# optozorax/portal

Hardware: AMD Instinct MI355X
Metric: Mray/s (primary rays) + ms/frame at 3840x2160, portal_in_portal depth=40 (higher is better)
Workload: dtype f32; 1 GPU; scenes/portal_in_portal.ron 3840x2160 aa=1 depth=40; build=w4, affine_rays=True, candidate_frames_identical=True, frames_in_flight=2, parallelism=row-block interleave x1, jit_specialisation=all scene uniforms baked (camera dynamic)

## Files before the change

### include/portal_amd.h

```cpp
#ifndef PORTAL_AMD_H
#define PORTAL_AMD_H

#include <stddef.h>
#include <stdint.h>

#ifdef __cplusplus
extern "C" {
#endif

#define PTL_OK 0
#define PTL_UNKNOWN_UNIFORM 1
#define PTL_ERR_INVALID (-1)
#define PTL_ERR_COMPILE (-2)
#define PTL_ERR_HIP (-3)
#define PTL_ERR_TYPE (-4)
#define PTL_ERR_SCENE (-5)
#define PTL_ERR_NO_DEVICE (-6)

const char* ptl_last_error(void);

const char* ptl_version(void);

int ptl_device_count(void);

// ... 20 lines not shown

int ptl_kernel_set_uniform(ptl_kernel* k, const char* name, ptl_type type, const void* value);

int ptl_kernel_set_texture(ptl_kernel* k, const char* sampler, const uint8_t* rgba8, int width, int height);

typedef struct {
    int width, height;
    int rb_phase, rb_stride;
    int in_place;
} ptl_frame;

int ptl_frame_shard_rows(const ptl_frame* f);

int ptl_kernel_render(ptl_kernel* k, const ptl_frame* frame, void* out_rgba8, void* out_rgba32f, void* segments,
                      void* stream, float* elapsed_ms);

int ptl_kernel_render_to_host(ptl_kernel* k, const ptl_frame* frame, uint8_t* host_rgba8, float* host_rgba32f,
                              uint64_t* host_segments, float* elapsed_ms);
int ptl_kernel_max_slices(ptl_kernel* k);
int ptl_kernel_stage_slice(ptl_kernel* k, int index);
int ptl_kernel_stage_slice_from(ptl_kernel* k, int index, const void* block, size_t size);
int ptl_kernel_hold_textures(ptl_kernel* k, int hold);
size_t ptl_kernel_uniform_block_size(ptl_kernel* k);
int ptl_kernel_snapshot_uniforms(ptl_kernel* k, void* dst, size_t cap);
int ptl_kernel_render_slices(ptl_kernel* k, const ptl_frame* frame, int n, void* out_rgba8, void* out_rgba32f, unsigned long long slice_pixels,
                             void* stream, float* elapsed_ms);

int ptl_kernel_teleport_ray(ptl_kernel* k, const float a[3], const float b[3], float out_pos[3], int* hit_object,
                            int* changed_subspace, int* teleported);
int ptl_kernel_prebuild_teleport(ptl_kernel* k);
// ... 45 lines not shown
#define PTL_FLAG_NO_FIRST_TRIP (1u << 13)
#define PTL_FLAG_EXACT_CR (1u << 14)
#define PTL_FLAG_NO_UNROLL (1u << 15)
#define PTL_FLAG_NO_FIRST_TRIP_PLANES (1u << 16)
#define PTL_FLAG_ASYNC_REJIT (1u << 17)
#define PTL_FLAG_QUICK_JIT (1u << 18)
#define PTL_FLAG_NO_ZERO_MASKS (1u << 19)
#define PTL_FLAG_SPECIALIZE_PATTERNS (1u << 20)
#define PTL_FLAG_BOUNDED_SNIPPETS (1u << 21)
#define PTL_FLAG_SLICES (1u << 22)
#define PTL_FLAG_NO_AFFINE_RAYS (1u << 23)
#define PTL_FLAG_KEEP_TRANSFORM_DODGES (1u << 24)
#define PTL_FLAG_CHECK_AFFINE (1u << 25)
#define PTL_FLAG_MATERIAL_TABLE_LDS (1u << 26)
#define PTL_FLAG_MATERIAL_TABLE_SCALAR (1u << 27)

int ptl_scene_generate_source(ptl_scene* s, unsigned flags, char** source);
int ptl_scene_generated_defines(ptl_scene* s, char* out, size_t cap);
int ptl_scene_zero_mask_probes(ptl_scene* s, int* reused, int* probed);
int ptl_scene_uniform_layout(ptl_scene* s, const ptl_uniform_desc** descs, int* n, size_t* block_size);
int ptl_scene_set_uniforms(ptl_scene* s, ptl_kernel* k);
typedef void (*ptl_uniform_cb)(void* user, const char* name, ptl_type type, const void* value);
int ptl_scene_visit_uniforms(ptl_scene* s, ptl_uniform_cb cb, void* user);
int ptl_scene_source_line_owner(ptl_scene* s, int line, char* kind, size_t kind_cap, char* name, size_t name_cap,
                                int* local_line);
void ptl_free(void* p);

int ptl_renderer_create(ptl_scene* s, int device, const char* asset_root, unsigned flags, ptl_renderer** out, char* log,
                        size_t log_cap);
int ptl_renderer_create_with_options(ptl_scene* s, int device, const char* asset_root, unsigned flags, const char* const* option_names,
// ... 103 lines not shown
```

### portal_amd/__init__.py

```python
from __future__ import annotations

import ctypes as C
import os
from typing import Callable, Optional

import numpy as np

_HERE = os.path.dirname(os.path.abspath(__file__))
REPO_ROOT = os.path.dirname(_HERE)
LIB_PATH = os.path.join(_HERE, "libportal_amd.so")

os.environ.setdefault("PTL_CACHE_DIR", os.path.join(_HERE, "_cache"))



def _share_torch_hip_runtime() -> None:
    if "PTL_HIP_LIB" in os.environ:
        return
    import importlib.util

    try:
        spec = importlib.util.find_spec("torch")
    except (ImportError, ValueError):
        spec = None
# ... 10 lines not shown
FLAG_SPECIALIZE_INTS = 1
FLAG_COUNT_SEGMENTS = 2
FLAG_SPECIALIZE_ALL = 4
FLAG_SPECIALIZE_STATIC = 8
FLAG_ANAGLYPH = 16
FLAG_NO_DERIVED_UNIFORMS = 32
FLAG_NO_FIRST_TRIP = 8192
FLAG_NO_UNIFORM_HOIST = 4096
FLAG_NO_DEFERRED_UPDATES = 128
FLAG_QUICK_JIT = 262144
FLAG_SPECIALIZE_PATTERNS = 1048576
FLAG_BOUNDED_SNIPPETS = 2097152
FLAG_KEEP_TRANSFORM_DODGES = 16777216
FLAG_MATERIAL_TABLE_LDS = 1 << 26
FLAG_MATERIAL_TABLE_SCALAR = 1 << 27
FLAG_CHECK_AFFINE = 1 << 25
FLAG_NO_AFFINE_RAYS = 8388608
FLAG_SLICES = 4194304
FLAG_NO_ZERO_MASKS = 524288
FLAG_ASYNC_REJIT = 131072
FLAG_NO_FIRST_TRIP_PLANES = 65536
FLAG_NO_UNROLL = 32768
FLAG_EXACT_CR = 16384
FLAG_FAST_MATH = 64


def flag_waves(n: int) -> int:
    return (int(n) & 0xF) << 8


class PortalError(RuntimeError):
    pass


class UniformDesc(C.Structure):
    _fields_ = [("name", C.c_char_p), ("type", C.c_int), ("offset", C.c_size_t)]


class CalculatedCam(C.Structure):
# ... 8 lines not shown


def _load() -> C.CDLL:
    if not os.path.exists(LIB_PATH):
        raise PortalError(f"{LIB_PATH} is missing: run `python -c 'import __graft_entry__ as g; g.build()'` or `make`")
    lib = C.CDLL(LIB_PATH)
    vp, cp, ci, cd, cs = C.c_void_p, C.c_char_p, C.c_int, C.c_double, C.c_size_t
    P = C.POINTER
    sig = {
        "ptl_last_error": (cp, []),
        "ptl_version": (cp, []),
        "ptl_device_count": (ci, []),
        "ptl_kernel_compile": (ci, [ci, cp, P(UniformDesc), ci, cs, P(cp), ci, P(vp), cp, cs]),
        "ptl_kernel_code_object": (ci, [vp, P(vp), P(cs)]),
        "ptl_kernel_resources": (ci, [vp, P(ci), P(ci), P(ci)]),
        "ptl_kernel_set_uniform": (ci, [vp, cp, ci, vp]),
        "ptl_kernel_set_texture": (ci, [vp, cp, vp, ci, ci]),
        "ptl_frame_shard_rows": (ci, [P(Frame)]),
        "ptl_kernel_render": (ci, [vp, P(Frame), vp, vp, vp, vp, P(C.c_float)]),
        "ptl_kernel_render_to_host": (ci, [vp, P(Frame), vp, vp, P(C.c_uint64), P(C.c_float)]),
        "ptl_kernel_teleport_ray": (ci, [vp, P(C.c_float), P(C.c_float), P(C.c_float), P(ci), P(ci), P(ci)]),
        "ptl_kernel_destroy": (None, [vp]),
        "ptl_scene_load_file": (ci, [cp, P(vp)]),
        "ptl_scene_load_text": (ci, [cp, P(vp)]),
        "ptl_scene_free": (None, [vp]),
        "ptl_scene_set_uniform": (ci, [vp, cp, cd]),
        "ptl_scene_set_time": (ci, [vp, cd, cd]),
        "ptl_scene_set_trefoil": (ci, [vp, cp, cp]),
        "ptl_scene_get_trefoil": (ci, [vp, cp, cp, cs]),
        "ptl_scene_init_stage": (ci, [vp, cp, cp, cs]),
# ... 378 lines not shown

    def teleport_external_ray(self, a, b):
        pa_, pb_, out = (C.c_double * 3)(*a), (C.c_double * 3)(*b), (C.c_double * 3)()
        hit, sub, tel = C.c_int(), C.c_int(), C.c_int()
        _check(lib().ptl_renderer_teleport_ray(self._h, pa_, pb_, out, C.byref(hit), C.byref(sub), C.byref(tel)), "teleport_external_ray")
        return (tuple(out) if tel.value else None), bool(hit.value), bool(sub.value)

    def prebuild_teleport(self) -> None:
        _check(lib().ptl_renderer_prebuild_teleport(self._h), "prebuild_teleport")

    def resources(self) -> dict:
        regs, scratch, lds = C.c_int(), C.c_int(), C.c_int()
        _check(lib().ptl_kernel_resources(lib().ptl_renderer_kernel(self._h), C.byref(regs), C.byref(scratch), C.byref(lds)), "kernel_resources")
        return {"registers": regs.value, "scratch_bytes": scratch.value, "lds_bytes": lds.value}

    def move_camera(self, look_at, alpha: float, beta: float, r: float):
        la, tel, blk = (C.c_double * 3)(*look_at), C.c_int(), C.c_int()
        _check(lib().ptl_renderer_move_camera(self._h, la, alpha, beta, r, C.byref(tel), C.byref(blk)), "move_camera")
        return bool(tel.value), bool(blk.value)

    def update(self, seconds: float):
        tel, blk = C.c_int(), C.c_int()
        _check(lib().ptl_renderer_update(self._h, float(seconds), C.byref(tel), C.byref(blk)), "update")
        return bool(tel.value), bool(blk.value)

    def rejit_count(self) -> int:
        return lib().ptl_renderer_rejit_count(self._h)

    def affine_rays(self) -> bool:
        lib().ptl_renderer_kernel(self._h)
# ... 315 lines not shown
```

### portal_amd/csrc/device/ptl_entry.h

```cpp

#if defined(PTL_NO_TELEPORT_ENTRY) && !defined(PTL_NO_DERIVE_ENTRY)
#define PTL_NO_DERIVE_ENTRY
#endif

#if PTL_DEVICE_BUILD

#ifdef PTL_WAVES_PER_EU
#define PTL_LAUNCH_BOUNDS __launch_bounds__(256, PTL_WAVES_PER_EU)
#else
#define PTL_LAUNCH_BOUNDS __launch_bounds__(256)
#endif

#if !defined(PTL_TELEPORT_MODULE)
extern "C" __global__ void PTL_LAUNCH_BOUNDS
ptl_render_kernel(unsigned int* __restrict__ out_rgba8,
                  float* __restrict__ out_rgba32f,
                  int width, int height,
                  int rb_phase, int rb_stride,
                  unsigned long long* __restrict__ segment_counter,
                  int in_place) {
#ifndef PTL_DIRECT_STORE
    __shared__ unsigned int tile[8][32 + 1];
#endif
    const int t = (int)threadIdx.x;
    const int wave = t >> 6, lane = t & 63;
    const int lx = wave * 8 + (lane & 7);
    const int ly = lane >> 3;
#ifdef PTL_XCD_SWIZZLE
// ... 167 lines not shown
```

### portal_amd/csrc/host/capi.cpp

```cpp
#include <chrono>
#include <cmath>
#include <cstdlib>
#include <cstring>
#include <map>
#include <memory>
#include <mutex>
#include <dirent.h>

#include <algorithm>
#include <atomic>
#include <set>
#include <thread>
#include <string>
#include <vector>

#include "../../../include/portal_amd.h"
#include "codegen.h"
#include "formula.h"
#include "glsl_hoist.h"
#include "glsl_translate.h"
#include "internal.h"
#include "scene.h"

using namespace ptl;
// ... 431 lines not shown
static KernelOptions options_from_flags(unsigned flags) {
    auto on = [flags](unsigned bit) { return (flags & bit) != 0; };
    KernelOptions o;
    o.specialize_ints = on(PTL_FLAG_SPECIALIZE_INTS);
    o.count_segments = on(PTL_FLAG_COUNT_SEGMENTS);
    o.specialize_all = on(PTL_FLAG_SPECIALIZE_ALL);
    o.anaglyph = on(PTL_FLAG_ANAGLYPH);
    o.specialize_static = on(PTL_FLAG_SPECIALIZE_STATIC);
    o.specialize_static_ints = on(PTL_FLAG_SPECIALIZE_PATTERNS);
    o.derived_uniforms = !on(PTL_FLAG_NO_DERIVED_UNIFORMS);
    o.fast_math = on(PTL_FLAG_FAST_MATH);
    o.exact_cr = on(PTL_FLAG_EXACT_CR);
    o.quick_jit = on(PTL_FLAG_QUICK_JIT) && !o.specialize_static;
    o.mask_zero_elements = specialised(flags) && !on(PTL_FLAG_NO_ZERO_MASKS);
    o.slices_entry = on(PTL_FLAG_SLICES);
    o.bound_snippets = on(PTL_FLAG_BOUNDED_SNIPPETS);
    const bool first_trip_forms = on(PTL_FLAG_KEEP_TRANSFORM_DODGES) || specialised(flags);
    o.first_trip_planes = first_trip_forms && !on(PTL_FLAG_NO_FIRST_TRIP_PLANES);
    if (const char* ab = std::getenv("PTL_AB_FIRST_TRIP_PLANES"); ab && (ab[0] == '0' || ab[0] == '1')) o.first_trip_planes = ab[0] == '1' && !on(PTL_FLAG_NO_FIRST_TRIP_PLANES);
    if (const char* skip = std::getenv("PTL_AFFINE_RAYS_SKIP_SCAN")) o.skip_affine_scan = skip[0] == '1';
    o.unroll_baked_loops = !on(PTL_FLAG_NO_UNROLL) && !o.quick_jit;
    o.keep_transform_dodges = on(PTL_FLAG_KEEP_TRANSFORM_DODGES);
    o.material_table = on(PTL_FLAG_MATERIAL_TABLE_SCALAR) ? 2 : (on(PTL_FLAG_MATERIAL_TABLE_LDS) ? 1 : 0);
    o.check_affine = on(PTL_FLAG_CHECK_AFFINE);
    o.affine_rays = !on(PTL_FLAG_NO_AFFINE_RAYS);
    o.first_trip = first_trip_forms && !on(PTL_FLAG_NO_FIRST_TRIP);
    o.hoist_uniform_work = !on(PTL_FLAG_NO_UNIFORM_HOIST);
    return o;
}

// ... 1394 lines not shown
```

### portal_amd/csrc/host/codegen.cpp

```cpp
#include "codegen.h"
#include "glsl_hoist.h"
#include "glsl_tokens.h"

#include <cstdlib>
#include <cstring>

#include <algorithm>
#include <charconv>
#include <cmath>
#include <cstdio>
#include <regex>
#include <set>
#include <sstream>
#include <tuple>

namespace ptl {

void LineNumbersByKey::offset(int lines) {
    for (auto& kv : ranges) {
        kv.second.start += lines;
        kv.second.end += lines;
    }
}
void LineNumbersByKey::add(const ElementKey& key, LineRange r) {
// ... 1463 lines not shown
    slots["uniforms"] = emit_uniforms(scene, plan, opts);
    std::tie(slots["material_processing"], slots["materials_defines"]) = emit_materials(scene, plan, opts);
    slots["intersection_functions"] = emit_intersection_functions(scene, plan, opts);
    slots["intersections"] = emit_intersections(scene, plan, opts, false);
    slots["intersections_first"] = plan.first_trip_plane_tests > 0 ? emit_intersections(scene, plan, opts, true) : StringStorage();
    slots["derive"] = emit_derive(scene, plan, opts);
    slots["intersection_material_functions"] = emit_intersection_material_functions(scene, plan, opts);
    slots["intersection_material_processing"] = emit_intersection_material_processing(scene, plan, opts, false);
    slots["intersection_material_processing_first"] = emit_intersection_material_processing(scene, plan, opts, true);
    slots["library"] = emit_library(scene, plan, opts);
    slots["predefined_library"] = emit_predefined_library(scene, plan, opts);
    slots["skybox_processing"] = emit_skybox_processing(scene, plan, opts);

    StringStorage body = apply_template(device_source_trace_template(), std::move(slots));
    body.add_string("\n");
    body.add_string(device_source_entry());
    GeneratedKernel gk = describe_kernel(plan, opts);
    gk.source = std::move(body.storage);
    gk.line_numbers = std::move(body.line_numbers);
    apply_zero_masks(gk.source, gk.masked);
    if (opts.slices_entry) apply_slices_entry(gk.source);
    return gk;
}

}
```

### portal_amd/csrc/host/codegen.h

```cpp
#pragma once
#include <map>
#include <set>
#include <string>
#include <vector>

#include "glsl_translate.h"
#include "scene.h"

namespace ptl {

struct ElementKey {
    std::string kind;
    std::string name;
    bool operator<(const ElementKey& o) const { return kind != o.kind ? kind < o.kind : name < o.name; }
    bool operator==(const ElementKey& o) const { return kind == o.kind && name == o.name; }
};
struct LineRange {
    int start = 0, end = 0;
};

class LineNumbersByKey {
public:
    std::map<ElementKey, LineRange> ranges;
    void offset(int lines);
// ... 54 lines not shown
    bool specialize_static = false;
    std::set<std::string> keep_dynamic;
    std::map<std::string, int> baked_options;
    bool mask_zero_elements = false;
    std::set<std::string> keep_unmasked;
    ZeroMaskCache* mask_cache = nullptr;
    bool full_chains = false;
    bool derived_uniforms = true;
    bool hoist_uniform_work = true;
    bool first_trip = true;
    bool unroll_baked_loops = true;
    bool exact_cr = false;
    bool first_trip_planes = true;
    bool bound_snippets = false;
    bool slices_entry = false;
    bool affine_rays = true;
    bool check_affine = false;
    bool skip_affine_scan = false;
    int material_table = 0;
    bool keep_transform_dodges = false;
    bool quick_jit = false;
    bool fast_math = false;
};

struct DerivedPlane {
    int object = 0, side = 0;
    std::string member;
    std::string normal_expr;
    std::string arg_expr;
};
// ... 42 lines not shown
```

### portal_amd/csrc/host/hip_api.cpp

```cpp
#ifndef _GNU_SOURCE
#define _GNU_SOURCE
#endif
#include "hip_api.h"

#include <stdlib.h>

#include <dlfcn.h>
#include <link.h>

#include <cstdlib>
#include <cstring>
#include <mutex>
#include <vector>

namespace ptl::hip {
namespace {

std::string loaded_library_path(const char* stem) {
    struct Ctx {
        const char* stem;
        std::string found;
    } ctx{stem, ""};
    dl_iterate_phdr(
        [](struct dl_phdr_info* info, size_t, void* data) -> int {
// ... 71 lines not shown
const Runtime* runtime(std::string* error) {
    static std::mutex mu;
    static Runtime rt;
    static bool tried = false, ok = false;
    static std::string err;
    std::lock_guard<std::mutex> lock(mu);
    if (!tried) {
        tried = true;
        const char* env = std::getenv("PTL_HIP_LIB");
        std::vector<std::string> candidates = {env ? env : "", loaded_library_path("libamdhip64.so"), "libamdhip64.so",
                                               "/opt/rocm/lib/libamdhip64.so"};
        void* h = open_first(candidates, &rt.path, &err);
        if (h) {
            ok = bind(h, "hipInit", rt.hipInit, &err) && bind(h, "hipGetDeviceCount", rt.hipGetDeviceCount, &err) &&
                 bind(h, "hipSetDevice", rt.hipSetDevice, &err) && bind(h, "hipGetDevice", rt.hipGetDevice, &err) &&
                 bind(h, "hipMalloc", rt.hipMalloc, &err) && bind(h, "hipFree", rt.hipFree, &err) &&
                 bind(h, "hipHostMalloc", rt.hipHostMalloc, &err) && bind(h, "hipHostFree", rt.hipHostFree, &err) &&
                 bind(h, "hipMemcpy", rt.hipMemcpy, &err) && bind(h, "hipMemcpyAsync", rt.hipMemcpyAsync, &err) &&
                 bind(h, "hipMemsetAsync", rt.hipMemsetAsync, &err) && bind(h, "hipStreamSynchronize", rt.hipStreamSynchronize, &err) &&
                 bind(h, "hipDeviceSynchronize", rt.hipDeviceSynchronize, &err) &&
                 bind(h, "hipStreamCreateWithFlags", rt.hipStreamCreateWithFlags, &err) && bind(h, "hipStreamDestroy", rt.hipStreamDestroy, &err) &&
                 bind(h, "hipStreamWaitEvent", rt.hipStreamWaitEvent, &err) && bind(h, "hipEventCreateWithFlags", rt.hipEventCreateWithFlags, &err) && bind(h, "hipEventCreate", rt.hipEventCreate, &err) &&
                 bind(h, "hipEventDestroy", rt.hipEventDestroy, &err) && bind(h, "hipEventRecord", rt.hipEventRecord, &err) &&
                 bind(h, "hipEventSynchronize", rt.hipEventSynchronize, &err) &&
                 bind(h, "hipEventElapsedTime", rt.hipEventElapsedTime, &err) && bind(h, "hipModuleLoadData", rt.hipModuleLoadData, &err) &&
                 bind(h, "hipModuleUnload", rt.hipModuleUnload, &err) && bind(h, "hipModuleGetFunction", rt.hipModuleGetFunction, &err) &&
                 bind(h, "hipModuleGetGlobal", rt.hipModuleGetGlobal, &err) && bind(h, "hipFuncGetAttribute", rt.hipFuncGetAttribute, &err) &&
                 bind(h, "hipModuleLaunchKernel", rt.hipModuleLaunchKernel, &err) && bind(h, "hipGetErrorString", rt.hipGetErrorString, &err) &&
                 bind(h, "hipIpcGetMemHandle", rt.hipIpcGetMemHandle, &err) && bind(h, "hipIpcOpenMemHandle", rt.hipIpcOpenMemHandle, &err) &&
                 bind(h, "hipIpcCloseMemHandle", rt.hipIpcCloseMemHandle, &err) && bind(h, "hipGetLastError", rt.hipGetLastError, &err) &&
// ... 63 lines not shown
```

### portal_amd/csrc/host/hip_api.h

```cpp
#pragma once
#include <cstddef>
#include <string>

namespace ptl::hip {

using hipError_t = int;
using hipStream_t = void*;
using hipEvent_t = void*;
using hipModule_t = void*;
using hipFunction_t = void*;
using hipDeviceptr_t = void*;
using hiprtcProgram = void*;
using hiprtcResult = int;

struct IpcMemHandle {
    char reserved[64];
};

struct Runtime {
    std::string path;
    hipError_t (*hipInit)(unsigned);
    hipError_t (*hipGetDeviceCount)(int*);
    hipError_t (*hipSetDevice)(int);
    hipError_t (*hipGetDevice)(int*);
    hipError_t (*hipMalloc)(void**, size_t);
    hipError_t (*hipFree)(void*);
    hipError_t (*hipHostMalloc)(void**, size_t, unsigned);
    hipError_t (*hipHostFree)(void*);
    hipError_t (*hipMemcpy)(void*, const void*, size_t, int);
    hipError_t (*hipMemcpyAsync)(void*, const void*, size_t, int, hipStream_t);
    hipError_t (*hipMemsetAsync)(void*, int, size_t, hipStream_t);
    hipError_t (*hipStreamSynchronize)(hipStream_t);
    hipError_t (*hipStreamCreateWithFlags)(hipStream_t*, unsigned);
    hipError_t (*hipStreamDestroy)(hipStream_t);
    hipError_t (*hipStreamWaitEvent)(hipStream_t, hipEvent_t, unsigned);
    hipError_t (*hipEventCreateWithFlags)(hipEvent_t*, unsigned);
    hipError_t (*hipDeviceSynchronize)();
    hipError_t (*hipEventCreate)(hipEvent_t*);
    hipError_t (*hipEventDestroy)(hipEvent_t);
// ... 5 lines not shown
    hipError_t (*hipModuleGetFunction)(hipFunction_t*, hipModule_t, const char*);
    hipError_t (*hipModuleGetGlobal)(hipDeviceptr_t*, size_t*, hipModule_t, const char*);
    hipError_t (*hipFuncGetAttribute)(int*, int, hipFunction_t);
    hipError_t (*hipModuleLaunchKernel)(hipFunction_t, unsigned, unsigned, unsigned, unsigned, unsigned, unsigned, unsigned,
                                        hipStream_t, void**, void**);
    const char* (*hipGetErrorString)(hipError_t);
    hipError_t (*hipIpcGetMemHandle)(IpcMemHandle*, void*);
    hipError_t (*hipIpcOpenMemHandle)(void**, IpcMemHandle, unsigned);
    hipError_t (*hipIpcCloseMemHandle)(void*);
    hipError_t (*hipGetLastError)();
    hipError_t (*hipDeviceCanAccessPeer)(int*, int, int);
    hipError_t (*hipDeviceEnablePeerAccess)(int, unsigned);
    hipError_t (*hipMemcpy2DAsync)(void*, size_t, const void*, size_t, size_t, size_t, int, hipStream_t);
};
constexpr int kFuncAttrSharedSizeBytes = 1, kFuncAttrLocalSizeBytes = 3, kFuncAttrNumRegs = 4;
constexpr unsigned kStreamNonBlocking = 1, kEventDisableTiming = 2, kIpcMemLazyEnablePeerAccess = 1;
constexpr int kMemcpyHostToDevice = 1;
constexpr int kMemcpyDeviceToHost = 2;
constexpr int kMemcpyDefault = 4;
constexpr int kErrorPeerAccessAlreadyEnabled = 704;

struct Rtc {
    std::string path;
    std::string real_path;
    hiprtcResult (*hiprtcCreateProgram)(hiprtcProgram*, const char*, const char*, int, const char**, const char**);
    hiprtcResult (*hiprtcCompileProgram)(hiprtcProgram, int, const char**);
    hiprtcResult (*hiprtcGetProgramLogSize)(hiprtcProgram, size_t*);
    hiprtcResult (*hiprtcGetProgramLog)(hiprtcProgram, char*);
    hiprtcResult (*hiprtcGetCodeSize)(hiprtcProgram, size_t*);
    hiprtcResult (*hiprtcGetCode)(hiprtcProgram, char*);
// ... 28 lines not shown
```

### portal_amd/csrc/host/kernel.cpp

```cpp
#include <sys/stat.h>
#include <unistd.h>

#include <cstdio>
#include <cstdlib>
#include <cstring>
#include <atomic>
#include <fstream>
#include <iterator>
#include <memory>
#include <map>
#include <string>
#include <vector>

#include "../../../include/portal_amd.h"
#include "hip_api.h"
#include "internal.h"

namespace ptl {

thread_local std::string g_last_error;
void set_last_error(const std::string& msg) { g_last_error = msg; }

namespace {

// ... 138 lines not shown
    std::vector<void*> retired_textures;
    bool staged_since_launch = false;
    int texture_holds = 0;
    hip::hipEvent_t ev0 = nullptr, ev1 = nullptr;
    hip::hipEvent_t ev_done = nullptr;
    bool sliced = false;
    bool affine_rays = false;
    hip::hipFunction_t derive_slices_fn = nullptr;
    void* dev_slices = nullptr;
    std::vector<unsigned char> staged;
    bool slice0_dirty = true;
    bool split = false;
    std::string source;
    std::vector<std::string> defines;
    ptl_kernel* companion = nullptr;
    unsigned block_waves = 4;
    void* last_stream = nullptr;
    bool launched = false;
};

extern "C" const char* ptl_last_error(void) { return g_last_error.c_str(); }

extern "C" const char* ptl_version(void) {
    static std::string v;
    std::string e1, e2;
    const hip::Runtime* rt = hip::runtime(&e1);
    const hip::Rtc* rc = hip::rtc(&e2);
    std::string toolchain = "?";
    if (rc) {
        size_t so = rc->real_path.rfind(".so.");
// ... 10 lines not shown
    if (rt->hipGetDeviceCount(&n) != 0) return 0;
    return n;
}

static constexpr int kMaxSlices = 16;

static size_t type_size(ptl_type t) {
    switch (t) {
        case PTL_MAT4: return 64;
        case PTL_F32: case PTL_I32: return 4;
        case PTL_VEC2: return 8;
        case PTL_VEC3: return 12;
        case PTL_SAMPLER: return 16;
    }
    return 0;
}

static thread_local bool tl_skip_cache_read = false;
static thread_local const std::vector<char>* tl_prebuilt_code = nullptr;

extern "C" int ptl_kernel_compile_prebuilt(int device, const char* hip_source, const ptl_uniform_desc* uniforms, int n_uniforms, size_t uniform_block_size,
                                           const char* const* defines, int n_defines, const void* code, size_t code_size, ptl_kernel** out, char* log,
                                           size_t log_cap) {
    if (!code || code_size < 64) return PTL_ERR_INVALID;
    const std::vector<char> copy(static_cast<const char*>(code), static_cast<const char*>(code) + code_size);
    tl_prebuilt_code = &copy;
    const int rc = ptl_kernel_compile(device, hip_source, uniforms, n_uniforms, uniform_block_size, defines, n_defines, out, log, log_cap);
    tl_prebuilt_code = nullptr;
    return rc;
}
// ... 11 lines not shown
    k->device = device;
    for (int i = 0; i < n_uniforms; ++i) {
        k->slots[uniforms[i].name] = {uniforms[i].type, uniforms[i].offset};
        if (uniforms[i].offset + type_size(uniforms[i].type) > uniform_block_size) {
            set_last_error(std::string("uniform `") + uniforms[i].name + "` lies outside the block");
            return PTL_ERR_INVALID;
        }
    }
    k->shadow.assign(uniform_block_size, 0);

    bool teleport_only = false;
    for (int i = 0; i < n_defines; ++i) {
        if (std::string(defines[i]) == "PTL_AFFINE_RAYS") k->affine_rays = true;
        if (std::string(defines[i]) == "PTL_RENDER_MODULE") k->split = true;
        if (std::string(defines[i]) == "PTL_TELEPORT_MODULE") teleport_only = true;
    }
    if (k->split) {
        k->source = hip_source;
        for (int i = 0; i < n_defines; ++i) k->defines.push_back(defines[i]);
    }
    std::vector<std::string> opts = compile_options(defines, n_defines);
    std::string cdir = cache_dir();
    std::string cache_path;
    if (!cdir.empty()) {
        unsigned long long h = fnv1a(hip_source);
        for (auto& o : opts) h = fnv1a(o, h);
        h = fnv1a("jit policy 6: occupancy retries end with an -O1 attempt", h);
        std::string err;
        if (const hip::Rtc* rc = hip::rtc(&err)) {
            h = fnv1a("hiprtc " + rc->real_path, h);
// ... 139 lines not shown
    }
    if (rt->hipModuleGetFunction(&k->derive_fn, k->module, "ptl_derive_kernel") != 0) {
        k->derive_fn = nullptr;
        rt->hipGetLastError();
    }
    if (!hip_ok(rt, rt->hipModuleGetGlobal(&k->dev_block, &k->dev_block_size, k->module, "_ZN4glsl5ptl_uE"), "hipModuleGetGlobal(ptl_u)"))
        return PTL_ERR_HIP;
    if (k->dev_block_size < uniform_block_size) {
        set_last_error("uniform block in the code object is smaller than the declared layout");
        return PTL_ERR_INVALID;
    }
    rt->hipEventCreate(&k->ev0);
    rt->hipEventCreate(&k->ev1);
    rt->hipEventCreateWithFlags(&k->ev_done, hip::kEventDisableTiming);
    if (const char* e = std::getenv("PTL_BLOCK_WAVES")) k->block_waves = (e[0] == '1' || e[0] == '2') ? (unsigned)(e[0] - '0') : 4u;
    *out = k.release();
    return PTL_OK;
}

extern "C" int ptl_kernel_clone(ptl_kernel* src, ptl_kernel** out) {
    if (!src || !out) return PTL_ERR_INVALID;
    if (src->device < 0 || !src->fn) return PTL_ERR_NO_DEVICE;
    const hip::Runtime* rt = hip::runtime(nullptr);
    if (!rt) return PTL_ERR_NO_DEVICE;
    auto k = std::make_unique<ptl_kernel>();
    k->device = src->device;
    k->code = src->code;
    k->slots = src->slots;
    k->shadow = src->shadow;
    k->block_waves = src->block_waves;
    k->split = src->split;
    k->source = src->source;
    k->defines = src->defines;
    if (!hip_ok(rt, rt->hipSetDevice(k->device), "hipSetDevice")) return PTL_ERR_HIP;
    if (!hip_ok(rt, rt->hipModuleLoadData(&k->module, k->code.data()), "hipModuleLoadData(clone)")) return PTL_ERR_HIP;
    auto fail = [&](int rc) {
        rt->hipModuleUnload(k->module);
        k->module = nullptr;
        return rc;
    };
    if (rt->hipModuleGetFunction(&k->fn, k->module, src->sliced ? "ptl_render_slices_kernel" : "ptl_render_kernel") != 0 ||
        (src->sliced && rt->hipModuleGetFunction(&k->derive_slices_fn, k->module, "ptl_derive_slices_kernel") != 0)) {
        hip_ok(rt, 1, "hipModuleGetFunction(clone)");
        return fail(PTL_ERR_HIP);
    }
    k->sliced = src->sliced;
    if (rt->hipModuleGetFunction(&k->teleport_fn, k->module, "ptl_teleport_kernel") != 0) {
        k->teleport_fn = nullptr;
        rt->hipGetLastError();
    }
    if (rt->hipModuleGetFunction(&k->derive_fn, k->module, "ptl_derive_kernel") != 0) {
        k->derive_fn = nullptr;
        rt->hipGetLastError();
    }
    if (!hip_ok(rt, rt->hipModuleGetGlobal(&k->dev_block, &k->dev_block_size, k->module, "_ZN4glsl5ptl_uE"), "hipModuleGetGlobal(ptl_u)")) return fail(PTL_ERR_HIP);
    rt->hipEventCreate(&k->ev0);
    rt->hipEventCreate(&k->ev1);
    rt->hipEventCreateWithFlags(&k->ev_done, hip::kEventDisableTiming);
    k->dirty = true;
    *out = k.release();
    return PTL_OK;
}

extern "C" int ptl_kernel_copy_uniforms(ptl_kernel* dst, const ptl_kernel* src) {
    if (!dst || !src || dst->shadow.size() != src->shadow.size()) return PTL_ERR_INVALID;
    if (std::memcmp(dst->shadow.data(), src->shadow.data(), src->shadow.size()) != 0) {
        dst->shadow = src->shadow;
        dst->dirty = true;
        dst->slice0_dirty = true;
    }
    return PTL_OK;
}

extern "C" int ptl_kernel_code_object(ptl_kernel* k, const void** data, size_t* size) {
    if (!k) return PTL_ERR_INVALID;
    if (data) *data = k->code.data();
    if (size) *size = k->code.size();
// ... 232 lines not shown
    if (k->device < 0 || !k->fn) return PTL_ERR_NO_DEVICE;
    const hip::Runtime* rt = hip::runtime(nullptr);
    if (!hip_ok(rt, rt->hipSetDevice(k->device), "hipSetDevice")) return PTL_ERR_HIP;
    if (k->sliced) {
        if (int rc = upload_slices(k, rt, stream, 1, true); rc != PTL_OK) return rc;
        return launch_slices(k, rt, frame, 1, out_rgba8, out_rgba32f, 0, segments, stream, elapsed_ms);
    }
    if (int rc = upload_uniforms(k, rt, stream); rc != PTL_OK) return rc;
    int nby = shard_blocks(frame);
    if (nby == 0) {
        if (elapsed_ms) *elapsed_ms = 0.0f;
        return PTL_OK;
    }
    int width = frame->width, height = frame->height, phase = frame->rb_phase, stride = frame->rb_stride;
    int in_place = frame->in_place ? 1 : 0;
    void* args[] = {&out_rgba8, &out_rgba32f, &width, &height, &phase, &stride, &segments, &in_place};
    const unsigned waves = k->block_waves;
    unsigned gx = (unsigned)((width + 8 * waves - 1) / (8 * waves)), gy = (unsigned)nby;
    if (elapsed_ms) rt->hipEventRecord(k->ev0, stream);
    if (!hip_ok(rt, rt->hipModuleLaunchKernel(k->fn, gx, gy, 1, 64 * waves, 1, 1, 0, stream, args, nullptr), "hipModuleLaunchKernel")) return PTL_ERR_HIP;
    k->last_stream = stream;
    k->launched = true;
    if (k->ev_done) rt->hipEventRecord(k->ev_done, stream);
    if (elapsed_ms) {
        rt->hipEventRecord(k->ev1, stream);
        if (!hip_ok(rt, rt->hipEventSynchronize(k->ev1), "hipEventSynchronize")) return PTL_ERR_HIP;
        rt->hipEventElapsedTime(elapsed_ms, k->ev0, k->ev1);
    }
    return PTL_OK;
}

extern "C" int ptl_kernel_render_to_host(ptl_kernel* k, const ptl_frame* frame, uint8_t* host_rgba8, float* host_rgba32f,
                                         uint64_t* host_segments, float* elapsed_ms) {
    if (!k || !frame) return PTL_ERR_INVALID;
    int rows = ptl_frame_shard_rows(frame);
// ... 93 lines not shown
    return PTL_OK;
}

extern "C" void ptl_kernel_destroy(ptl_kernel* k) {
    if (!k) return;
    if (k->companion) ptl_kernel_destroy(k->companion);
    const hip::Runtime* rt = k->device >= 0 ? hip::runtime(nullptr) : nullptr;
    if (rt) {
        rt->hipSetDevice(k->device);
        if (k->launched && k->ev_done) rt->hipEventSynchronize(k->ev_done);
        if (k->ev_done) rt->hipEventDestroy(k->ev_done);
        for (auto& t : k->textures)
            if (t.second) rt->hipFree(t.second);
        free_retired_textures(k, rt);
        if (k->dev_slices) rt->hipFree(k->dev_slices);
        if (k->ev0) rt->hipEventDestroy(k->ev0);
        if (k->ev1) rt->hipEventDestroy(k->ev1);
        if (k->module) rt->hipModuleUnload(k->module);
    }
    delete k;
}

extern "C" int ptl_deinterleave_rows(const uint8_t* shard, const ptl_frame* f, uint8_t* full) {
    if (!shard || !f || !full || ptl_frame_shard_rows(f) < 0) return PTL_ERR_INVALID;
    int blocks = (f->height + 7) / 8;
    size_t pitch = (size_t)f->width * 4;
    size_t src_row = 0;
    for (int b = f->rb_phase; b < blocks; b += f->rb_stride) {
        for (int r = 0; r < 8 && b * 8 + r < f->height; ++r) {
            std::memcpy(full + (size_t)(b * 8 + r) * pitch, shard + src_row * pitch, pitch);
// ... 6 lines not shown
```

Before: 46990 Mray/s.

## Add persistent and work-queue render entry forms, default to persistent grid

Adds a persistent-threads kernel entry in which a grid sized from CU count, register and LDS occupancy loops over 32x8 pixel blocks. A second form pulls chunks of blocks from a global atomic ticket queue. Persistent is now the default. The goal is to cut workgroup launch and dispatch overhead and to balance divergent per-block portal-trace cost. The trade-off is static striding that can leave CUs idle at the tail, plus extra LDS double-buffering and barriers per block for the rgba8 writeback.

```diff
diff --git a/include/portal_amd.h b/include/portal_amd.h
--- a/include/portal_amd.h
+++ b/include/portal_amd.h
@@ -58,6 +58,14 @@
 
 int ptl_kernel_render(ptl_kernel* k, const ptl_frame* frame, void* out_rgba8, void* out_rgba32f, void* segments,
                       void* stream, float* elapsed_ms);
+
+#define PTL_ENTRY_FORM_GRID 0
+#define PTL_ENTRY_FORM_PERSISTENT 1
+#define PTL_ENTRY_FORM_QUEUE 2
+#define PTL_DEFAULT_ENTRY PTL_ENTRY_FORM_PERSISTENT
+#define PTL_ENTRY_QUEUE_CHUNK 4
+int ptl_kernel_entry_form(ptl_kernel* k);
+int ptl_persistent_grid(int blocks, int chunk, int cu_count, int registers, int lds_bytes, int* resident_per_cu);
 
 int ptl_kernel_render_to_host(ptl_kernel* k, const ptl_frame* frame, uint8_t* host_rgba8, float* host_rgba32f,
                               uint64_t* host_segments, float* elapsed_ms);
@@ -133,6 +141,9 @@
 #define PTL_FLAG_CHECK_AFFINE (1u << 25)
 #define PTL_FLAG_MATERIAL_TABLE_LDS (1u << 26)
 #define PTL_FLAG_MATERIAL_TABLE_SCALAR (1u << 27)
+#define PTL_FLAG_ENTRY_GRID (1u << 28)
+#define PTL_FLAG_ENTRY_PERSISTENT (1u << 29)
+#define PTL_FLAG_ENTRY_QUEUE (1u << 30)
 
 int ptl_scene_generate_source(ptl_scene* s, unsigned flags, char** source);
 int ptl_scene_generated_defines(ptl_scene* s, char* out, size_t cap);
diff --git a/portal_amd/__init__.py b/portal_amd/__init__.py
--- a/portal_amd/__init__.py
+++ b/portal_amd/__init__.py
@@ -48,6 +48,9 @@
 FLAG_KEEP_TRANSFORM_DODGES = 16777216
 FLAG_MATERIAL_TABLE_LDS = 1 << 26
 FLAG_MATERIAL_TABLE_SCALAR = 1 << 27
+FLAG_ENTRY_GRID = 1 << 28
+FLAG_ENTRY_PERSISTENT = 1 << 29
+FLAG_ENTRY_QUEUE = 1 << 30
 FLAG_CHECK_AFFINE = 1 << 25
 FLAG_NO_AFFINE_RAYS = 8388608
 FLAG_SLICES = 4194304
@@ -57,6 +60,15 @@
 FLAG_NO_UNROLL = 32768
 FLAG_EXACT_CR = 16384
 FLAG_FAST_MATH = 64
+
+
+ENTRY_FORM_GRID, ENTRY_FORM_PERSISTENT, ENTRY_FORM_QUEUE = 0, 1, 2
+ENTRY_QUEUE_CHUNK = 4
+
+
+def persistent_grid(blocks: int, chunk: int, cu_count: int, registers: int, lds_bytes: int):
+    k = C.c_int()
+    return lib().ptl_persistent_grid(blocks, chunk, cu_count, registers, lds_bytes, C.byref(k)), k.value
 
 
 def flag_waves(n: int) -> int:
@@ -95,6 +107,8 @@
         "ptl_kernel_compile": (ci, [ci, cp, P(UniformDesc), ci, cs, P(cp), ci, P(vp), cp, cs]),
         "ptl_kernel_code_object": (ci, [vp, P(vp), P(cs)]),
         "ptl_kernel_resources": (ci, [vp, P(ci), P(ci), P(ci)]),
+        "ptl_kernel_entry_form": (ci, [vp]),
+        "ptl_persistent_grid": (ci, [ci, ci, ci, ci, ci, P(ci)]),
         "ptl_kernel_set_uniform": (ci, [vp, cp, ci, vp]),
         "ptl_kernel_set_texture": (ci, [vp, cp, vp, ci, ci]),
         "ptl_frame_shard_rows": (ci, [P(Frame)]),
@@ -503,6 +517,9 @@
         _check(lib().ptl_kernel_resources(lib().ptl_renderer_kernel(self._h), C.byref(regs), C.byref(scratch), C.byref(lds)), "kernel_resources")
         return {"registers": regs.value, "scratch_bytes": scratch.value, "lds_bytes": lds.value}
 
+    def entry_form(self) -> int:
+        return lib().ptl_kernel_entry_form(lib().ptl_renderer_kernel(self._h))
+
     def move_camera(self, look_at, alpha: float, beta: float, r: float):
         la, tel, blk = (C.c_double * 3)(*look_at), C.c_int(), C.c_int()
         _check(lib().ptl_renderer_move_camera(self._h, la, alpha, beta, r, C.byref(tel), C.byref(blk)), "move_camera")
diff --git a/portal_amd/csrc/device/ptl_entry.h b/portal_amd/csrc/device/ptl_entry.h
--- a/portal_amd/csrc/device/ptl_entry.h
+++ b/portal_amd/csrc/device/ptl_entry.h
@@ -11,7 +11,144 @@
 #define PTL_LAUNCH_BOUNDS __launch_bounds__(256)
 #endif
 
-#if !defined(PTL_TELEPORT_MODULE)
+#if !defined(PTL_TELEPORT_MODULE) && defined(PTL_PERSISTENT_ENTRY)
+typedef unsigned int ptl_u32x4 __attribute__((ext_vector_type(4)));
+struct ptl_entry_args {
+    unsigned int* out_rgba8;
+    float* out_rgba32f;
+    int width, height, rb_phase, rb_stride;
+    unsigned long long* segment_counter;
+    int in_place, blocks_x, blocks_y;
+    unsigned long long* queue_head;
+    unsigned long long queue_base;
+};
+static_assert(__builtin_offsetof(ptl_entry_args, segment_counter) == 32 && __builtin_offsetof(ptl_entry_args, blocks_x) == 44 &&
+              __builtin_offsetof(ptl_entry_args, queue_head) == 56 && sizeof(ptl_entry_args) == 72, "kernel-argument layout");
+#define PTL_ENTRY_ARGS_AS __attribute__((address_space(4)))
+PTL_FN const PTL_ENTRY_ARGS_AS ptl_entry_args& ptl_entry_arguments() {
+    int ptl_zero = 0;
+    asm volatile("" : "+s"(ptl_zero));
+    return *(const PTL_ENTRY_ARGS_AS ptl_entry_args*)((const PTL_ENTRY_ARGS_AS char*)__builtin_amdgcn_kernarg_segment_ptr() + ptl_zero);
+}
+extern "C" __global__ void PTL_LAUNCH_BOUNDS ptl_render_kernel(
+        unsigned int* __restrict__, float* __restrict__, int, int, int, int,
+        unsigned long long* __restrict__, int,
+        int, int,
+        unsigned long long* __restrict__, unsigned long long) {
+    __shared__ __attribute__((aligned(16))) unsigned int tile[2][8][32 + 4];
+    const int t = (int)threadIdx.x;
+
+#ifdef PTL_COUNT_SEGMENTS
+    ptl_segments_lds[t] = 0u;
+#endif
+#if defined(PTL_MATERIAL_TABLE) && PTL_MATERIAL_TABLE == 1
+    {
+        for (int k = (int)threadIdx.x; k < PTL_MATERIAL_TABLE_WORDS; k += (int)blockDim.x) glsl::ptl_material_table[k] = glsl::ptl_material_table_init[k];
+        __syncthreads();
+    }
+#endif
+#ifdef PTL_UNIFORMS_IN_LDS
+    {
+        const unsigned int* src = reinterpret_cast<const unsigned int*>(&glsl::ptl_u);
+        unsigned int* dst = reinterpret_cast<unsigned int*>(&glsl::ptl_lds_u);
+        for (int i = t; i < (int)(sizeof(glsl::ptl_uniform_block) / 4); i += 256) dst[i] = src[i];
+        __syncthreads();
+    }
+#endif
+    unsigned int turn = 0;
+    auto render_block = [&](const int id) __attribute__((always_inline)) {
+        int block_x, block_y;
+        glsl::vec4 c = glsl::vec4(0.0f);
+        {
+            int tb = t;
+            asm volatile("" : "+v"(tb));
+            const int lx = (tb >> 6) * 8 + (tb & 7), ly = (tb & 63) >> 3;
+            const PTL_ENTRY_ARGS_AS ptl_entry_args& a = ptl_entry_arguments();
+            block_y = __builtin_amdgcn_readfirstlane(id / a.blocks_x);
+            block_x = __builtin_amdgcn_readfirstlane(id - block_y * a.blocks_x);
+            const int px = block_x * 32 + lx;
+            const int py = (a.rb_phase + block_y * a.rb_stride) * 8 + ly;
+            if (px < a.width && py < a.height) c = glsl::shade_pixel(glsl::vec2((float)px + 0.5f, (float)py + 0.5f));
+        }
+        int ta = t;
+        asm volatile("" : "+s"(block_x), "+s"(block_y), "+v"(ta));
+        const int wave = ta >> 6, lane = ta & 63;
+        const int lx = wave * 8 + (lane & 7), ly = lane >> 3;
+        const PTL_ENTRY_ARGS_AS ptl_entry_args& a = ptl_entry_arguments();
+        unsigned int* const out_rgba8 = a.out_rgba8;
+        float* const out_rgba32f = a.out_rgba32f;
+        const int width = a.width, height = a.height;
+        const int frame_block = a.rb_phase + block_y * a.rb_stride;
+        const int px = block_x * 32 + lx;
+        const bool live = px < width && frame_block * 8 + ly < height;
+        const int out_block = a.in_place ? frame_block : block_y;
+        if (out_rgba32f != nullptr && live) {
+            float4 v = make_float4(c.x, c.y, c.z, c.w);
+            *reinterpret_cast<float4*>(out_rgba32f + 4 * (((long)out_block * 8 + ly) * width + px)) = v;
+        }
+        if (out_rgba8 != nullptr) {
+            unsigned int(*const rows)[32 + 4] = tile[turn & 1u];
+            rows[ly][lx] = glsl::pack_rgba8(c);
+            __syncthreads();
+            if (wave == (int)(turn & 3u)) {
+                const int gy0 = frame_block * 8;
+                if ((width & 3) == 0 && (reinterpret_cast<unsigned long long>(out_rgba8) & 15ull) == 0) {
+                    const int row = lane >> 3, gx = block_x * 32 + (lane & 7) * 4;
+                    if (gx < width && gy0 + row < height)
+                        __builtin_nontemporal_store(*reinterpret_cast<const ptl_u32x4*>(&rows[row][(lane & 7) * 4]),
+                                                    reinterpret_cast<ptl_u32x4*>(out_rgba8 + ((long)out_block * 8 + row) * width + gx));
+                } else {
+                    for (int k = 0; k < 4; ++k) {
+                        const int row = k * 2 + (lane >> 5), col = lane & 31, gx = block_x * 32 + col;
+                        if (gx < width && gy0 + row < height) out_rgba8[((long)out_block * 8 + row) * width + gx] = rows[row][col];
+                    }
+                }
+            }
+        }
+        ++turn;
+    };
+    auto block_count = [&]() __attribute__((always_inline)) {
+        const PTL_ENTRY_ARGS_AS ptl_entry_args& a = ptl_entry_arguments();
+        return a.blocks_x * a.blocks_y;
+    };
+#ifdef PTL_ENTRY_QUEUE
+    __shared__ unsigned int ticket_slot[2];
+    auto draw_ticket = [&]() __attribute__((always_inline)) {
+        const PTL_ENTRY_ARGS_AS ptl_entry_args& a = ptl_entry_arguments();
+        return (unsigned int)(__hip_atomic_fetch_add(a.queue_head, 1ull, __ATOMIC_RELAXED, __HIP_MEMORY_SCOPE_AGENT) - a.queue_base);
+    };
+    if (t == 0) ticket_slot[0] = draw_ticket();
+    __syncthreads();
+    unsigned int parity = 0;
+    unsigned int chunk = __builtin_amdgcn_readfirstlane(ticket_slot[0]);
+    while ((long)chunk * PTL_ENTRY_QUEUE < (long)block_count()) {
+        unsigned int next = 0;
+        if (t == 0) next = draw_ticket();
+        for (int k = 0; k < PTL_ENTRY_QUEUE; ++k) {
+            const int id = (int)chunk * PTL_ENTRY_QUEUE + k;
+            if (id >= block_count()) break;
+            render_block(id);
+        }
+        parity ^= 1u;
+        if (t == 0) ticket_slot[parity] = next;
+        __syncthreads();
+        chunk = __builtin_amdgcn_readfirstlane(ticket_slot[parity]);
+    }
+#else
+    for (int id = (int)blockIdx.x; id < block_count(); id += (int)gridDim.x) render_block(id);
+#endif
+#ifdef PTL_COUNT_SEGMENTS
+    {
+        unsigned long long* const segment_counter = ptl_entry_arguments().segment_counter;
+        if (segment_counter != nullptr) {
+            unsigned int n = ptl_segments_lds[t];
+            for (int off = 32; off > 0; off >>= 1) n += __shfl_down(n, off, 64);
+            if ((t & 63) == 0) atomicAdd(segment_counter, (unsigned long long)n);
+        }
+    }
+#endif
+}
+#elif !defined(PTL_TELEPORT_MODULE)
 extern "C" __global__ void PTL_LAUNCH_BOUNDS
 ptl_render_kernel(unsigned int* __restrict__ out_rgba8,
                   float* __restrict__ out_rgba32f,
diff --git a/portal_amd/csrc/host/capi.cpp b/portal_amd/csrc/host/capi.cpp
--- a/portal_amd/csrc/host/capi.cpp
+++ b/portal_amd/csrc/host/capi.cpp
@@ -469,6 +469,9 @@
     o.quick_jit = on(PTL_FLAG_QUICK_JIT) && !o.specialize_static;
     o.mask_zero_elements = specialised(flags) && !on(PTL_FLAG_NO_ZERO_MASKS);
     o.slices_entry = on(PTL_FLAG_SLICES);
+    o.render_entry = on(PTL_FLAG_ENTRY_GRID) ? PTL_ENTRY_FORM_GRID : on(PTL_FLAG_ENTRY_QUEUE) ? PTL_ENTRY_FORM_QUEUE : on(PTL_FLAG_ENTRY_PERSISTENT) ? PTL_ENTRY_FORM_PERSISTENT : PTL_DEFAULT_ENTRY;
+    o.entry_queue_chunk = PTL_ENTRY_QUEUE_CHUNK;
+    if (const char* bw = std::getenv("PTL_BLOCK_WAVES"); bw && (bw[0] == '1' || bw[0] == '2')) o.render_entry = PTL_ENTRY_FORM_GRID;
     o.bound_snippets = on(PTL_FLAG_BOUNDED_SNIPPETS);
     const bool first_trip_forms = on(PTL_FLAG_KEEP_TRANSFORM_DODGES) || specialised(flags);
     o.first_trip_planes = first_trip_forms && !on(PTL_FLAG_NO_FIRST_TRIP_PLANES);
diff --git a/portal_amd/csrc/host/codegen.cpp b/portal_amd/csrc/host/codegen.cpp
--- a/portal_amd/csrc/host/codegen.cpp
+++ b/portal_amd/csrc/host/codegen.cpp
@@ -1501,6 +1501,10 @@
 
     StringStorage body = apply_template(device_source_trace_template(), std::move(slots));
     body.add_string("\n");
+    if (opts.render_entry != 0 && !opts.slices_entry) {
+        body.add_string("#define PTL_PERSISTENT_ENTRY 1\n");
+        if (opts.render_entry == 2) body.add_string("#define PTL_ENTRY_QUEUE " + std::to_string(std::max(1, opts.entry_queue_chunk)) + "\n");
+    }
     body.add_string(device_source_entry());
     GeneratedKernel gk = describe_kernel(plan, opts);
     gk.source = std::move(body.storage);
diff --git a/portal_amd/csrc/host/codegen.h b/portal_amd/csrc/host/codegen.h
--- a/portal_amd/csrc/host/codegen.h
+++ b/portal_amd/csrc/host/codegen.h
@@ -92,6 +92,8 @@
     bool first_trip_planes = true;
     bool bound_snippets = false;
     bool slices_entry = false;
+    int render_entry = 0;
+    int entry_queue_chunk = 4;
     bool affine_rays = true;
     bool check_affine = false;
     bool skip_affine_scan = false;
diff --git a/portal_amd/csrc/host/hip_api.cpp b/portal_amd/csrc/host/hip_api.cpp
--- a/portal_amd/csrc/host/hip_api.cpp
+++ b/portal_amd/csrc/host/hip_api.cpp
@@ -109,6 +109,7 @@
         if (h) {
             ok = bind(h, "hipInit", rt.hipInit, &err) && bind(h, "hipGetDeviceCount", rt.hipGetDeviceCount, &err) &&
                  bind(h, "hipSetDevice", rt.hipSetDevice, &err) && bind(h, "hipGetDevice", rt.hipGetDevice, &err) &&
+                 bind(h, "hipDeviceGetAttribute", rt.hipDeviceGetAttribute, &err) &&
                  bind(h, "hipMalloc", rt.hipMalloc, &err) && bind(h, "hipFree", rt.hipFree, &err) &&
                  bind(h, "hipHostMalloc", rt.hipHostMalloc, &err) && bind(h, "hipHostFree", rt.hipHostFree, &err) &&
                  bind(h, "hipMemcpy", rt.hipMemcpy, &err) && bind(h, "hipMemcpyAsync", rt.hipMemcpyAsync, &err) &&
diff --git a/portal_amd/csrc/host/hip_api.h b/portal_amd/csrc/host/hip_api.h
--- a/portal_amd/csrc/host/hip_api.h
+++ b/portal_amd/csrc/host/hip_api.h
@@ -23,6 +23,7 @@
     hipError_t (*hipGetDeviceCount)(int*);
     hipError_t (*hipSetDevice)(int);
     hipError_t (*hipGetDevice)(int*);
+    hipError_t (*hipDeviceGetAttribute)(int*, int, int);
     hipError_t (*hipMalloc)(void**, size_t);
     hipError_t (*hipFree)(void*);
     hipError_t (*hipHostMalloc)(void**, size_t, unsigned);
@@ -58,6 +59,7 @@
     hipError_t (*hipMemcpy2DAsync)(void*, size_t, const void*, size_t, size_t, size_t, int, hipStream_t);
 };
 constexpr int kFuncAttrSharedSizeBytes = 1, kFuncAttrLocalSizeBytes = 3, kFuncAttrNumRegs = 4;
+constexpr int kDeviceAttrMultiprocessorCount = 63;
 constexpr unsigned kStreamNonBlocking = 1, kEventDisableTiming = 2, kIpcMemLazyEnablePeerAccess = 1;
 constexpr int kMemcpyHostToDevice = 1;
 constexpr int kMemcpyDeviceToHost = 2;
diff --git a/portal_amd/csrc/host/kernel.cpp b/portal_amd/csrc/host/kernel.cpp
--- a/portal_amd/csrc/host/kernel.cpp
+++ b/portal_amd/csrc/host/kernel.cpp
@@ -4,6 +4,7 @@
 #include <cstdio>
 #include <cstdlib>
 #include <cstring>
+#include <algorithm>
 #include <atomic>
 #include <fstream>
 #include <iterator>
@@ -176,6 +177,11 @@
     std::string source;
     std::vector<std::string> defines;
     ptl_kernel* companion = nullptr;
+    int entry_form = PTL_ENTRY_FORM_GRID;
+    int queue_chunk = 1;
+    int cu_count = 0, entry_registers = 0, entry_lds = 0;
+    void* dev_queue = nullptr;
+    unsigned long long queue_next = 0;
     unsigned block_waves = 4;
     void* last_stream = nullptr;
     bool launched = false;
@@ -216,6 +222,52 @@
         case PTL_SAMPLER: return 16;
     }
     return 0;
+}
+
+extern "C" int ptl_persistent_grid(int blocks, int chunk, int cu_count, int registers, int lds_bytes, int* resident_per_cu) {
+    int k = 8;
+    if (registers > 0) k = std::min(k, std::max(1, 512 / ((registers + 7) / 8 * 8)));
+    if (lds_bytes > 0) k = std::min(k, std::max(1, 160 * 1024 / lds_bytes));
+    if (resident_per_cu) *resident_per_cu = k;
+    if (blocks <= 0) return 0;
+    if (chunk < 1) chunk = 1;
+    const long units = ((long)blocks + chunk - 1) / chunk;
+    long grid = cu_count > 0 ? std::min(units, (long)k * cu_count) : units;
+    if (grid >= 8) grid -= grid % 8;
+    return (int)grid;
+}
+
+static int define_value(const char* source, const char* const* defines, int n_defines, const std::string& name) {
+    auto number = [](const char* p) {
+        while (*p == ' ') ++p;
+        return (*p >= '0' && *p <= '9') ? std::max(1, std::atoi(p)) : 1;
+    };
+    for (int i = 0; i < n_defines; ++i) {
+        const std::string d = defines[i];
+        if (d == name) return 1;
+        if (d.compare(0, name.size() + 1, name + "=") == 0) return number(d.c_str() + name.size() + 1);
+    }
+    const std::string line = "#define " + name;
+    for (const char* at = source; (at = std::strstr(at, line.c_str())) != nullptr; at += line.size()) {
+        const char after = at[line.size()];
+        if ((at == source || at[-1] == '\n') && (after == ' ' || after == '\n' || after == '\0')) return number(at + line.size());
+    }
+    return 0;
+}
+
+static bool prepare_persistent(ptl_kernel* k, const hip::Runtime* rt) {
+    if (k->entry_form == PTL_ENTRY_FORM_GRID || !k->fn) return true;
+    int v = 0;
+    k->cu_count = rt->hipDeviceGetAttribute(&v, hip::kDeviceAttrMultiprocessorCount, k->device) == 0 ? v : 0;
+    k->entry_registers = std::max(code_object_note_max(k->code, ".vgpr_count", "ptl_render"), rt->hipFuncGetAttribute(&v, hip::kFuncAttrNumRegs, k->fn) == 0 ? v : 0);
+    k->entry_lds = rt->hipFuncGetAttribute(&v, hip::kFuncAttrSharedSizeBytes, k->fn) == 0 ? v : 0;
+    if (k->entry_form == PTL_ENTRY_FORM_QUEUE) {
+        const unsigned long long zero = 0;
+        if (!hip_ok(rt, rt->hipMalloc(&k->dev_queue, sizeof zero), "hipMalloc(block queue)")) return false;
+        if (!hip_ok(rt, rt->hipMemcpy(k->dev_queue, &zero, sizeof zero, hip::kMemcpyHostToDevice), "hipMemcpy(block queue)")) return false;
+        k->queue_next = 0;
+    }
+    return true;
 }
 
 static thread_local bool tl_skip_cache_read = false;
@@ -257,6 +309,11 @@
         if (std::string(defines[i]) == "PTL_AFFINE_RAYS") k->affine_rays = true;
         if (std::string(defines[i]) == "PTL_RENDER_MODULE") k->split = true;
         if (std::string(defines[i]) == "PTL_TELEPORT_MODULE") teleport_only = true;
+    }
+    if (define_value(hip_source, defines, n_defines, "PTL_PERSISTENT_ENTRY")) {
+        k->queue_chunk = define_value(hip_source, defines, n_defines, "PTL_ENTRY_QUEUE");
+        k->entry_form = k->queue_chunk ? PTL_ENTRY_FORM_QUEUE : PTL_ENTRY_FORM_PERSISTENT;
+        if (!k->queue_chunk) k->queue_chunk = 1;
     }
     if (k->split) {
         k->source = hip_source;
@@ -426,6 +483,12 @@
     rt->hipEventCreate(&k->ev1);
     rt->hipEventCreateWithFlags(&k->ev_done, hip::kEventDisableTiming);
     if (const char* e = std::getenv("PTL_BLOCK_WAVES")) k->block_waves = (e[0] == '1' || e[0] == '2') ? (unsigned)(e[0] - '0') : 4u;
+    if (k->sliced) k->entry_form = PTL_ENTRY_FORM_GRID;
+    if (k->entry_form != PTL_ENTRY_FORM_GRID && k->block_waves != 4) {
+        set_last_error("PTL_BLOCK_WAVES: the persistent render entry is written for 256-thread workgroups; generate the grid form (PTL_FLAG_ENTRY_GRID)");
+        return PTL_ERR_INVALID;
+    }
+    if (!prepare_persistent(k.get(), rt)) return PTL_ERR_HIP;
     *out = k.release();
     return PTL_OK;
 }
@@ -441,6 +504,8 @@
     k->slots = src->slots;
     k->shadow = src->shadow;
     k->block_waves = src->block_waves;
+    k->entry_form = src->entry_form;
+    k->queue_chunk = src->queue_chunk;
     k->split = src->split;
     k->source = src->source;
     k->defines = src->defines;
@@ -470,9 +535,15 @@
     rt->hipEventCreate(&k->ev1);
     rt->hipEventCreateWithFlags(&k->ev_done, hip::kEventDisableTiming);
     k->dirty = true;
+    if (!prepare_persistent(k.get(), rt)) {
+        ptl_kernel_destroy(k.release());
+        return PTL_ERR_HIP;
+    }
     *out = k.release();
     return PTL_OK;
 }
+
+extern "C" int ptl_kernel_entry_form(ptl_kernel* k) { return k ? k->entry_form : PTL_ERR_INVALID; }
 
 extern "C" int ptl_kernel_copy_uniforms(ptl_kernel* dst, const ptl_kernel* src) {
     if (!dst || !src || dst->shadow.size() != src->shadow.size()) return PTL_ERR_INVALID;
@@ -735,11 +806,25 @@
     }
     int width = frame->width, height = frame->height, phase = frame->rb_phase, stride = frame->rb_stride;
     int in_place = frame->in_place ? 1 : 0;
-    void* args[] = {&out_rgba8, &out_rgba32f, &width, &height, &phase, &stride, &segments, &in_place};
     const unsigned waves = k->block_waves;
     unsigned gx = (unsigned)((width + 8 * waves - 1) / (8 * waves)), gy = (unsigned)nby;
+    int blocks_x = (int)gx, blocks_y = nby;
+    void* queue = k->dev_queue;
+    unsigned long long queue_base = k->queue_next, queue_taken = 0;
+    void* args[] = {&out_rgba8, &out_rgba32f, &width, &height, &phase, &stride, &segments, &in_place, &blocks_x, &blocks_y, &queue, &queue_base};
+    if (k->entry_form != PTL_ENTRY_FORM_GRID) {
+        if ((long)blocks_x * blocks_y > 0x7fffffffL) {
+            set_last_error("ptl_kernel_render: the frame has more 32x8 blocks than the persistent entry counts");
+            return PTL_ERR_INVALID;
+        }
+        const int blocks = blocks_x * blocks_y;
+        gx = (unsigned)ptl_persistent_grid(blocks, k->queue_chunk, k->cu_count, k->entry_registers, k->entry_lds, nullptr);
+        gy = 1;
+        if (k->entry_form == PTL_ENTRY_FORM_QUEUE) queue_taken = (unsigned long long)((blocks + k->queue_chunk - 1) / k->queue_chunk) + gx;
+    }
     if (elapsed_ms) rt->hipEventRecord(k->ev0, stream);
     if (!hip_ok(rt, rt->hipModuleLaunchKernel(k->fn, gx, gy, 1, 64 * waves, 1, 1, 0, stream, args, nullptr), "hipModuleLaunchKernel")) return PTL_ERR_HIP;
+    k->queue_next += queue_taken;
     k->last_stream = stream;
     k->launched = true;
     if (k->ev_done) rt->hipEventRecord(k->ev_done, stream);
@@ -863,6 +948,7 @@
             if (t.second) rt->hipFree(t.second);
         free_retired_textures(k, rt);
         if (k->dev_slices) rt->hipFree(k->dev_slices);
+        if (k->dev_queue) rt->hipFree(k->dev_queue);
         if (k->ev0) rt->hipEventDestroy(k->ev0);
         if (k->ev1) rt->hipEventDestroy(k->ev1);
         if (k->module) rt->hipModuleUnload(k->module);
```

New measurement: 45890 Mray/s. -2.3%, worse.
